# gergely-flamich/relative-entropy-coding

Measured on AMD Instinct MI355X. Metric: encoded latents/sec, higher is better.
Workload: dtype f32

## Files before the change

relative-entropy-coding_amd/csrc/irec_fast_common.h:

```cpp
#pragma once
#include <hip/hip_runtime.h>
#include <stdint.h>

#include "irec_device.h"
#include "irec_kernels.h"

namespace irec {

__device__ __forceinline__ int64_t src_index(const EncArgs &A, int64_t base, int32_t pos, int d) {
  return base + (A.perm ? (int64_t)A.perm[pos + d] : (int64_t)(pos + d));
}

__device__ __forceinline__ void commit_table_stamps(const EncArgs &A) {
  if (A.ws_head != nullptr && blockIdx.x == 0 && threadIdx.x < 4 * WS_STAMP_WORDS)
    A.ws_head[WS_STAMP_WORD + threadIdx.x] = A.ws_head[WS_PENDING_WORD + threadIdx.x];
}

__device__ __forceinline__ void plain_table_rows(int64_t seed, int32_t S, int32_t D, int32_t K_tab, const uint16_t *__restrict__ dlog4r,
                                                 uint16_t *__restrict__ tab, int64_t wg, int64_t n_wg) {
  const int Dp = (D + 3) & ~3;
  const int64_t per_step = (int64_t)S * Dp;
  const int64_t total = per_step * K_tab;
  for (int64_t q = (wg * 256 + threadIdx.x) * 4; q < total; q += n_wg * 256 * 4) {
    const int t = (int)(q / per_step);
    const int64_t rem = q - (int64_t)t * per_step;
    const int s = (int)(rem / Dp), d0 = (int)(rem - (int64_t)s * Dp);
    const StepSeed ss = make_step_seed(seed + t);
    uint16_t v[4];
#pragma unroll
    for (int i = 0; i < 4; ++i) v[i] = (d0 + i < D) ? dlog4r[draw_rm1(ss, (uint64_t)s * (uint64_t)D + (uint64_t)(d0 + i))] : (uint16_t)0;
    *reinterpret_cast<uint2 *>(tab + q) = make_uint2((uint32_t)v[0] | ((uint32_t)v[1] << 16), (uint32_t)v[2] | ((uint32_t)v[3] << 16));
  }
}

__device__ __forceinline__ unsigned long long stamp_now() { return __builtin_amdgcn_s_memtime(); }

template <int MB, int CPW = 32, int NC = 64>
struct SmallLdsT {
  static constexpr int CANDS = NC;
  static constexpr int CP = CPW;
  union {
    unsigned long long wb[32];
    unsigned long long cand[NC];
  };
  int32_t sel_s[MB], sel_b[MB];
  uint32_t sel_bo[MB];
  int32_t hsum[2][MB];
  uint32_t beta4[2][MB];
  int32_t misc[8];
  union {
    double gpart[4];
    float cpart[4][CPW];
  };
  float Cb[CPW];
};
using SmallLds = SmallLdsT<64>;
constexpr size_t SMALL_LDS_BYTES = (sizeof(SmallLds) + 15) & ~(size_t)15;

struct NoPost { __device__ __forceinline__ void operator()(int, int32_t, int32_t, uint32_t) const {} };
template <bool QUICK>
__device__ __forceinline__ uint32_t kth_largest_lane_max(uint32_t M, int Bnew) {
  uint32_t cnt_gt = 0u;
#pragma unroll
  for (int l = 0; l < 64; ++l) cnt_gt += (uint32_t)__builtin_amdgcn_readlane((int)M, l) > M ? 1u : 0u;
  if constexpr (!QUICK) {
    uint32_t T = cnt_gt < (uint32_t)Bnew ? M : 0xFFFFFFFFu;
    T = 0xFFFFFFFFu - (uint32_t)wave_max_u64((unsigned long long)(0xFFFFFFFFu - T));
    return T;
  }
  uint32_t T = 0u;
  for (int c = Bnew <= 64 ? Bnew - 1 : 63; c >= 0; --c) {
    const unsigned long long hit = __ballot(cnt_gt == (uint32_t)c);
    if (hit) { T = (uint32_t)__builtin_amdgcn_readlane((int)M, (int)__builtin_ctzll(hit)); break; }
  }
  return T;
}

template <bool QUICK, class SM, class Post>
__device__ __forceinline__ bool rank_survivors(SM *sm, uint32_t C, int Bnew, int Bcur, int tid, Post &&post) {
  constexpr int NQ = SM::CANDS / 64;
  if (C > (uint32_t)SM::CANDS || C < (uint32_t)Bnew) return false;
  if (C > 64u) {
    if constexpr (NQ > 1) {
      uint32_t mk[NQ], mf[NQ];
#pragma unroll
      for (int q = 0; q < NQ; ++q) {
        const uint32_t at = (uint32_t)(q * 64 + tid);
        const unsigned long long v = at < C ? sm->cand[at] : 0ull;
        mk[q] = (uint32_t)(v >> 32); mf[q] = (uint32_t)v;
      }
      uint32_t T2 = 0u;
      for (int bit = 31; bit >= 0; --bit) {
        const uint32_t tryT = T2 | (1u << bit);
        uint32_t cnt = 0u;
#pragma unroll
        for (int q = 0; q < NQ; ++q) cnt += (uint32_t)__popcll(__ballot(mk[q] >= tryT));
        if (cnt >= (uint32_t)Bnew) T2 = tryT;
      }
      uint32_t base = 0u;
#pragma unroll
      for (int q = 0; q < NQ; ++q) {
        const bool in = mk[q] >= T2 && mk[q] != 0u;
        const unsigned long long mask = __ballot(in);
        const uint32_t pos = base + __builtin_amdgcn_mbcnt_hi((uint32_t)(mask >> 32), __builtin_amdgcn_mbcnt_lo((uint32_t)mask, 0u));
        if (in && pos < 64u) sm->cand[pos] = ((unsigned long long)mk[q] << 32) | mf[q];
        base += (uint32_t)__popcll(mask);
      }
      C = (uint32_t)__builtin_amdgcn_readfirstlane((int)base);
      if (C > 64u) return false;
    } else {
      return false;
    }
  }
  const unsigned long long mine = tid < (int)C ? sm->cand[tid] : 0ull;
  const uint32_t mk1 = (uint32_t)(mine >> 32), mf1 = (uint32_t)mine;
  uint32_t rank = 0u;
  if constexpr (!QUICK) {
    for (uint32_t l = 0; l < C; ++l) {
      const uint32_t ok_ = (uint32_t)__builtin_amdgcn_readlane((int)mk1, (int)l);
      const uint32_t of_ = (uint32_t)__builtin_amdgcn_readlane((int)mf1, (int)l);
      rank += (ok_ > mk1 || (ok_ == mk1 && of_ < mf1)) ? 1u : 0u;
    }
  } else {
  const uint32_t nf1 = ~mf1;
  const unsigned long long mp = ((unsigned long long)mk1 << 32) | nf1;
#pragma unroll
  for (int l0 = 0; l0 < 64; l0 += 8) {
    if ((uint32_t)l0 < C) {
#pragma unroll
      for (int l = l0; l < l0 + 8; ++l) rank += (uint32_t)__builtin_amdgcn_readlane((int)mk1, l) > mk1 ? 1u : 0u;
    }
  }
  volatile unsigned long long *slot = sm->cand;
  if (tid < (int)C) slot[rank] = (unsigned long long)tid;
  const bool lost = tid < (int)C && slot[rank] != (unsigned long long)tid;
  if (__ballot(lost)) {
    rank = 0u;
// ... 377 lines not shown
__device__ __forceinline__ int rsn_owner(int lane) {
  int idx = 0, cnt = N0, n = N0;
#pragma unroll
  for (int dist = 32; dist >= 1; dist >>= 1) {
    if (n >= 2) {
      const int H = (n + 1) / 2;
      if (lane & dist) { idx += H; cnt -= H; } else cnt = cnt < H ? cnt : H;
      n = H;
    }
  }
  return cnt >= 1 ? idx : -1;
}

typedef float rs_f2 __attribute__((ext_vector_type(2)));
__device__ __forceinline__ float reduce_scatter_20(rs_f2 (&a)[10], int lane) {
  float w[5];
#pragma unroll
  for (int k = 0; k < 5; ++k) {
    float px = a[k].x, py = a[k].y, qx = a[k + 5].x, qy = a[k + 5].y;
    swap32(px, qx); swap32(py, qy);
    a[k] = (rs_f2){px, py} + (rs_f2){qx, qy};
  }
#pragma unroll
  for (int k = 0; k < 2; ++k) {
    float px = a[k].x, py = a[k].y, qx = a[k + 2].x, qy = a[k + 2].y;
    swap16(px, qx); swap16(py, qy);
    a[k] = (rs_f2){px, py} + (rs_f2){qx, qy};
  }
  float tx = a[4].x, ty = a[4].y;
  swap16(tx, ty);
  w[0] = a[0].x; w[1] = a[0].y; w[2] = a[1].x; w[3] = a[1].y; w[4] = tx + ty;
  float r0, r1, r2, q0, q1;
  asm("s_nop 1\n\t"
      "v_add_f32_dpp %0, %3, %3 row_ror:8 row_mask:0xf bank_mask:0x3\n\t"
      "v_add_f32_dpp %1, %4, %4 row_ror:8 row_mask:0xf bank_mask:0x3\n\t"
      "v_add_f32_dpp %2, %5, %5 row_ror:8 row_mask:0xf bank_mask:0xf\n\t"
      "v_add_f32_dpp %0, %6, %6 row_ror:8 row_mask:0xf bank_mask:0xc\n\t"
      "v_add_f32_dpp %1, %7, %7 row_ror:8 row_mask:0xf bank_mask:0xc"
      : "=&v"(r0), "=&v"(r1), "=&v"(r2) : "v"(w[0]), "v"(w[1]), "v"(w[2]), "v"(w[3]), "v"(w[4]));
  asm("s_nop 1\n\t"
      "v_add_f32_dpp %0, %2, %2 row_shl:4 row_mask:0xf bank_mask:0x5\n\t"
      "v_add_f32_dpp %1, %3, %3 row_shl:4 row_mask:0xf bank_mask:0xf\n\t"
      "v_add_f32_dpp %0, %4, %4 row_shr:4 row_mask:0xf bank_mask:0xa"
      : "=&v"(q0), "=&v"(q1) : "v"(r0), "v"(r1), "v"(r2));
  float s0, s1, tot;
  asm("s_nop 1\n\t"
      "v_add_f32_dpp %0, %2, %2 quad_perm:[2,3,0,1] row_mask:0xf bank_mask:0xf\n\t"
      "v_add_f32_dpp %1, %3, %3 quad_perm:[2,3,0,1] row_mask:0xf bank_mask:0xf"
      : "=&v"(s0), "=&v"(s1) : "v"(q0), "v"(q1));
  const float kept = (lane & 2) ? s1 : s0;
  asm("s_nop 1\n\t"
      "v_add_f32_dpp %0, %1, %1 quad_perm:[1,0,3,2] row_mask:0xf bank_mask:0xf"
      : "=&v"(tot) : "v"(kept));
  return tot;
}
__device__ __forceinline__ int rs20_owner(int lane) {
  int o5 = 0, cnt = 5, n = 5;
#pragma unroll
  for (int dist = 8; dist >= 1; dist >>= 1) {
    if (n >= 2) {
      const int H = (n + 1) / 2;
      if (lane & dist) { o5 += H; cnt -= H; } else cnt = cnt < H ? cnt : H;
      n = H;
    }
  }
  if (cnt < 1) return -1;
  const int hi16 = (lane >> 4) & 1;
  const int v10 = o5 < 4 ? o5 + 4 * hi16 : 8 + hi16;
  return v10 + ((lane & 32) ? 10 : 0);
}

typedef __attribute__((address_space(3))) const float lds_cfloat;
__device__ __forceinline__ float lds_abs_f32(uint32_t byte_addr) { return *(lds_cfloat *)(uintptr_t)(byte_addr); }

template <int NB, bool TABLE>
struct FastCfg {
  static constexpr int RW = NB <= 10 ? 64 : 32;
  static constexpr int SPC = RW / NB;
  static_assert(SPC >= 1, "NB too large");
};

__host__ __device__ inline size_t fast_ws_bytes(int NB, int max_K) {
  const size_t bp = (((size_t)(max_K > 0 ? max_K : 1) * NB * 4) + 255) & ~(size_t)255;
  return bp + (size_t)5 * FAST_MAX_DIM * 4 + (size_t)2 * NB * FAST_MAX_DIM * 4;
}

}
```

relative-entropy-coding_amd/csrc/irec_team.hip:

```cpp
#include <hip/hip_runtime.h>
#include <algorithm>
#include <stdint.h>
#include <stdio.h>

#include "irec_device.h"
#include "irec_kernels.h"
#include "irec_fast_common.h"
#include "irec_team_common.h"

#ifndef IREC_GANG_ABLATE
#define IREC_GANG_ABLATE 0
#endif
#ifndef IREC_PK_ADDR
#define IREC_PK_ADDR 1
#endif
#if defined(IREC_TEAM_MARGIN_TU) || defined(IREC_TEAM_GANG_TU)
#define IREC_TEAM_AUX_TU 1
#endif
namespace irec {

__host__ __device__ constexpr int team_mb(int NB) { return NB <= 32 ? 32 : 64; }
template <int NB> using TeamLdsT = SmallLdsT<(NB <= 32 ? 32 : 64), (NB <= 32 ? 32 : 64), (NB <= 32 ? 64 : 512)>;
__host__ __device__ inline size_t team_small_bytes(int NB) {
  return NB <= 32 ? ((sizeof(TeamLdsT<32>) + 15) & ~(size_t)15) : ((sizeof(TeamLdsT<64>) + 15) & ~(size_t)15);
// ... 56 lines not shown
  const int S = A.S, B = A.B;
  const int lane = threadIdx.x & 63;
  const int wave_wg = __builtin_amdgcn_readfirstlane((int)(threadIdx.x >> 6));
  const int team = wave_wg / NWT, wave_t = wave_wg % NWT;
  const int wave = wave_t & 3, bs = wave_t >> 2;
  const int b_lo = bs * NBW;
  const int tid = (int)threadIdx.x - team * NT;
  const int PS = NB == 10 ? team_row(NB, B) : NB;
  const int SP = MULTI_PASS ? team_s_pass(NB, S, TEAMS, CMAX, PASSES, PS) : S;
  const bool keys_lds = !MULTI_PASS || team_keys_in_lds(NB, S, TEAMS, PASSES, PS);
  constexpr bool KEYS_ALIAS = TEAMS >= 3 && NB == 20 && !PASSES;
  const size_t key_lds_bytes = (keys_lds && !KEYS_ALIAS) ? team_key_bytes(PS, S) : 0;
  char *tbase = smem + T3_BYTES + (size_t)team * team_lds_one(NB, S, SP, TEAMS, PASSES, PS);
  float *part_s = reinterpret_cast<float *>(tbase);
  TeamLds *sm = reinterpret_cast<TeamLds *>(tbase + team_part_bytes(PS, SP) + key_lds_bytes);
  uint32_t *bar_word = reinterpret_cast<uint32_t *>(tbase + team_part_bytes(PS, SP) + key_lds_bytes + TEAM_SMALL_BYTES);
  double *gpart = sm->gpart;
  int32_t *sel_s = sm->sel_s, *sel_b = sm->sel_b;
  int32_t *hsum = &sm->hsum[0][0];
  uint32_t *beta4 = &sm->beta4[0][0];
  int32_t *misc = sm->misc;
  float *cpart_s = &sm->cpart[0][0];
  const uint16_t *dlog_s = A.dlog4r;
  const int rs_p = rsn_owner<RW>(lane);
  const int rs_p20 = RW == 20 ? rs20_owner(lane) : -1;
  const int rs_c = rsn_owner<NBW>(lane);

  if ((uint32_t)(uintptr_t)(__attribute__((address_space(3))) char *)smem != 0u) __builtin_trap();
  commit_table_stamps(A);
  constexpr bool CAN_SHARE = SHARE && TEAMS >= 2 && BS == 1 && !PASSES && !ONE;
  const int Wsh = (CAN_SHARE && A.coop_W > 1) ? A.coop_W : 1;
  const int64_t n_whole = Wsh > 1 ? (A.tsplit_first < A.n_blocks ? A.tsplit_first : A.n_blocks) : A.n_blocks;
  const int64_t n_slots = n_whole + (A.n_blocks - n_whole) * Wsh;
  const int64_t n_static = (int64_t)TEAMS * (int64_t)gridDim.x < n_slots ? (int64_t)TEAMS * (int64_t)gridDim.x : n_slots;
  constexpr bool CAN_PLACE = NB == 20 && TEAMS == 2 && BS == 1 && !PASSES && !ONE;
  const bool placed = CAN_PLACE && A.row_cost != nullptr && n_static == n_slots;
  const int64_t lo_rank = (int64_t)gridDim.x < n_whole ? (int64_t)gridDim.x : n_whole;
  int32_t placed_row = -1;
  if (placed) {
    uint32_t *cs = reinterpret_cast<uint32_t *>(smem);
    const int n = (int)A.n_blocks;
    for (int k = (int)threadIdx.x; k < n; k += TEAMS * NT) cs[k] = A.row_cost[k];
    if ((int)threadIdx.x < TEAMS) cs[n + (int)threadIdx.x] = 0xFFFFFFFFu;
    int want[TEAMS];
#pragma unroll
    for (int tm = 0; tm < TEAMS; ++tm) {
      const int64_t u = (int64_t)tm * (int64_t)gridDim.x + (int64_t)blockIdx.x;
      want[tm] = u >= n_static ? -1 : u < lo_rank ? (int)u : n - 1 - (int)((u - lo_rank) / (u < n_whole ? 1 : Wsh));
    }
    __syncthreads();
    for (int i = (int)threadIdx.x; i < n; i += TEAMS * NT) {
      const uint32_t ci = cs[i];
      int rk = 0;
#pragma unroll 8
      for (int j = 0; j < n; ++j) rk += cs[j] < ci ? 1 : 0;
#pragma unroll
      for (int tm = 0; tm < TEAMS; ++tm)
        if (rk == want[tm]) cs[n + tm] = (uint32_t)i;
    }
    __syncthreads();
    placed_row = (int32_t)cs[n + team];
    __syncthreads();
  }
  {
    float *l3 = reinterpret_cast<float *>(smem);
    for (int k = (int)threadIdx.x; k < (int)IREC_PM1; k += TEAMS * NT) {
      const float v = A.lut2[k];
      l3[k] = v; l3[k + IREC_PM1] = v; l3[k + 2 * IREC_PM1] = v;
    }
    if (tid == 0) *bar_word = 0u;
  }
  __syncthreads();
  TeamBarrier tsync{bar_word, 0u, (uint32_t)NWT};

  char *slab = A.ws + ((size_t)blockIdx.x * TEAMS + team) * A.ws_per_wg;
  const size_t key_glb_bytes = keys_lds ? 0 : ((team_key_bytes(PS, S) + 255) & ~(size_t)255);
  uint32_t *key_s = KEYS_ALIAS ? reinterpret_cast<uint32_t *>(tbase)
                    : keys_lds ? reinterpret_cast<uint32_t *>(tbase + team_part_bytes(PS, SP))
                               : reinterpret_cast<uint32_t *>(slab + A.ws_per_wg - key_glb_bytes);
  int32_t *bp = reinterpret_cast<int32_t *>(slab);
  float *beams_g = reinterpret_cast<float *>(slab + A.ws_per_wg - key_glb_bytes - (size_t)2 * NB * FAST_MAX_DIM * 4);
  float *stats_g = beams_g - 3 * FAST_MAX_DIM;
  float *park_g = stats_g - 2 * FAST_MAX_DIM;
  constexpr bool PARK = SHORT;
  constexpr bool LATE_G = false;

#ifdef IREC_TEAM_STAMPS
  unsigned long long st_acc[12] = {0, 0, 0, 0, 0, 0, 0, 0, 0, 0, 0, 0};
  unsigned long long st_prev = __builtin_amdgcn_s_memtime();
  const unsigned long long st_t0 = st_prev, st_r0 = __builtin_amdgcn_s_memrealtime();
#endif
  bool first_block = true;
  int steal = 0;
  for (;;) {
    tsync();
    if (tid == 0) {
      int64_t r;
      if (first_block) {
        r = (int64_t)team * (int64_t)gridDim.x + (int64_t)blockIdx.x;
        r = r < n_static ? (placed ? r : xcd_static_row(r, n_static, (int)gridDim.x)) : n_slots;
      } else r = placed ? n_slots : xcd_pull_row(A, n_static, n_slots, steal);
      misc[0] = (int32_t)r;
      misc[6] = 0;
    }
    first_block = false;
    tsync();
    const int64_t slot = misc[0];
    TSTAMP(0);
    if (slot >= n_slots) break;
    int64_t blk = slot < n_whole ? slot : n_whole + (slot - n_whole) / Wsh;
    const int64_t xrow = slot < n_whole ? 0 : (slot - n_whole) / Wsh;
    const int qsh = slot < n_whole ? 0 : (int)((slot - n_whole) % Wsh);
    const int Wrow = slot < n_whole ? 1 : Wsh;
    if (placed) {
      blk = placed_row;
      if (blk < 0 || blk >= A.n_blocks) __builtin_trap();
    }
    if (Wrow > 1 && A.coop_test_orphan && qsh != 0) continue;
    const int D = A.block_dim[blk];
    const int64_t base = A.block_base[blk];
    const int32_t pos = A.block_pos[blk];
    const uint16_t *tab = nullptr;
#pragma unroll
    for (int q = 0; q < 4; ++q)
      if (A.tab_dim[q] == D) tab = A.tab[q];
    if (D < 1 || D > FAST_MAX_DIM || tab == nullptr) {
      if (tid == 0 && qsh == 0) A.out_K[blk] = -1;
      continue;
    }
    const int Dp = (D + 3) & ~3;
    const int NG = (D + 255) >> 8;
    const int NSW = NW / NG;
    const bool active = wave < NG * NSW;
    const int g = wave % NG, sw = wave / NG;
    const int NSWe = NSW * Wrow, swe = sw * Wrow + qsh;
    const int d0 = g * 256 + lane * 4;

    float c[4];
    bool valid[4];
    float own_dmu[4], own_vq[4], own_vp[4];
    const bool own_stats = active && sw == 0 && bs == 0 && TEAMS < 3 && !SHORT;
    double klacc = 0.0;
#pragma unroll
    for (int i = 0; i < 4; ++i) {
      const int d = d0 + i;
      valid[i] = d < D;
      c[i] = 0.f;
      const int64_t ixi = valid[i] ? src_index(A, base, pos, d) : src_index(A, base, pos, 0);
      float st3[3] = {0.f, 1.f, 1.f};
      if (valid[i] && active && sw == 0 && bs == 0) {
        const float mq_ = A.q_loc[ixi], sq_ = A.q_scale[ixi], mp_ = A.p_loc[ixi], sp_ = A.p_scale[ixi];
        klacc = klacc + kl_dim(mq_, sq_, mp_, sp_);
        st3[0] = mq_ - mp_; st3[1] = sq_ * sq_; st3[2] = sp_ * sp_;
      }
      own_dmu[i] = st3[0]; own_vq[i] = st3[1]; own_vp[i] = st3[2];
      if (active && sw == 0 && bs == 0 && (NSW > 1 || BS > 1 || TEAMS >= 3)) {
        stats_g[d0 + i] = st3[0]; stats_g[FAST_MAX_DIM + d0 + i] = st3[1]; stats_g[2 * FAST_MAX_DIM + d0 + i] = st3[2];
      }
    }
    {
      const double gs = wave_tree_sum(klacc);
      if (sw == 0 && bs == 0 && active && lane == 0) gpart[g] = gs;
      tsync();
      if (tid == 0) {
        double tot = gpart[0];
        for (int gg = 1; gg < NG; ++gg) tot = tot + gpart[gg];
        const int32_t K = num_aux((float)tot, A.omega);
        misc[1] = K;
        if (qsh == 0) A.out_K[blk] = K;
        hsum[0] = 0;
        beta4[0] = 0u;
        if constexpr (MARGIN) { if (qsh == 0) margin_write(A.out_margin, blk, MarginAcc()); }
      }
      tsync();
    }
    const int K = misc[1];
    MarginAcc macc;
    if (K > A.max_K || K > A.K_limit) continue;
    if (K > A.K_tab) {
      if (tid == 0 && qsh == 0) atomicAdd(A.defer_count, 1u);
      continue;
    }
    if (K == 0) {
      if (active && sw == 0 && bs == 0 && qsh == 0) {
#pragma unroll
        for (int i = 0; i < 4; ++i)
          if (valid[i]) { const int64_t ixo = src_index(A, base, pos, d0 + i); A.out_sample[ixo] = 0.f + A.p_loc[ixo]; }
      }
      continue;
    }

    float sa[4], cH[4];
    float G[NBW][4];
    auto step_consts = [&](int t_next, float (&m)[4], float (&cA)[4], float (&cBv)[4]) {
      const float rho = A.rho[K - 1 - t_next];
      float dmu_[4], vq_[4], vp_[4];
      if (own_stats) {
#pragma unroll
        for (int i = 0; i < 4; ++i) { dmu_[i] = own_dmu[i]; vq_[i] = own_vq[i]; vp_[i] = own_vp[i]; }
      } else {
        const float4 q0 = *reinterpret_cast<const float4 *>(stats_g + d0);
        const float4 q1 = *reinterpret_cast<const float4 *>(stats_g + FAST_MAX_DIM + d0);
        const float4 q2 = *reinterpret_cast<const float4 *>(stats_g + 2 * FAST_MAX_DIM + d0);
        dmu_[0] = q0.x; dmu_[1] = q0.y; dmu_[2] = q0.z; dmu_[3] = q0.w;
        vq_[0] = q1.x; vq_[1] = q1.y; vq_[2] = q1.z; vq_[3] = q1.w;
        vp_[0] = q2.x; vp_[1] = q2.y; vp_[2] = q2.z; vp_[3] = q2.w;
      }
#pragma unroll
      for (int i = 0; i < 4; ++i) {
        const StepConst sc = step_constants(rho, dmu_[i], vq_[i], vp_[i], c[i]);
        sa[i] = valid[i] ? sc.sa : 0.f; cH[i] = valid[i] ? sc.H : 0.f;
        m[i] = valid[i] ? sc.m : 0.f; cA[i] = valid[i] ? sc.A : 0.f; cBv[i] = valid[i] ? sc.Bv : 0.f;
        c[i] = c[i] + sc.a;
        __builtin_amdgcn_sched_barrier(0);
      }
    };
    auto park = [&]() {
      if (PARK && active) {
        *reinterpret_cast<float4 *>(park_g + d0) = make_float4(c[0], c[1], c[2], c[3]);
        *reinterpret_cast<float4 *>(park_g + FAST_MAX_DIM + d0) = make_float4(sa[0], sa[1], sa[2], sa[3]);
      }
    };
    auto unpark = [&]() {
      if (PARK && active) {
        asm volatile("" ::: "memory");
        const float4 pc = *reinterpret_cast<const float4 *>(park_g + d0);
        const float4 ps = *reinterpret_cast<const float4 *>(park_g + FAST_MAX_DIM + d0);
        c[0] = pc.x; c[1] = pc.y; c[2] = pc.z; c[3] = pc.w;
        sa[0] = ps.x; sa[1] = ps.y; sa[2] = ps.z; sa[3] = ps.w;
      }
    };
    {
      float m[4], cA[4], cBv[4];
      step_consts(0, m, cA, cBv);
      park();
      float cacc = 0.f;
#pragma unroll
      for (int b = 0; b < NBW; ++b)
#pragma unroll
        for (int i = 0; i < 4; ++i) G[b][i] = 0.f;
#pragma unroll
      for (int i = 0; i < 4; ++i) {
        if (bs == 0) G[0][i] = beam_G(0.f, m[i], cA[i], cBv[i], sa[i]);
        cacc = beam_C_term(cacc, 0.f, m[i], cA[i], cBv[i]);
      }
      const float cg = wave_tree_sum(cacc);
      if (active && sw == 0 && bs == 0 && lane == 0) cpart_s[g * TEAM_MB + 0] = cg;
    }

    TSTAMP(1);
    bool abandoned = false;
    int cur = 0, Bcur = 1;
    uint32_t bv_cur = 0u;
    for (int t = 0; t < K; ++t) {
#ifdef IREC_TEAM_STAMPS
      st_acc[11] += 1ull;
#endif
      const uint16_t *tab_tu = tab + (size_t)t * S * Dp;
      const uint32_t tab_lo = (uint32_t)(d0 < Dp ? d0 : Dp - 4);
      const uint16_t *tab_t = tab_tu + tab_lo;
      uint32_t bet[NBW];
      {
#pragma unroll
        for (int b = 0; b < NBW; ++b) bet[b] = (uint32_t)__builtin_amdgcn_readlane((int)bv_cur, b_lo + b);
      }
      const int nlive = Bcur - b_lo < 0 ? 0 : (Bcur - b_lo < NBW ? Bcur - b_lo : NBW);

      const int N = S * Bcur;
      for (int s_base = 0; s_base < S; s_base += SP) {
      const int s_end = s_base + SP < S ? s_base + SP : S;
      const int Sp = s_end - s_base;
#ifdef IREC_ABLATE_SCORING
      if (false) {
#else
      if (active && Bcur > 1 && (nlive == NBW || 2 * nlive >= NBW)) {
        const int n_mine = Sp > swe ? (Sp - swe + NSWe - 1) / NSWe : 0;
        const int n_chunks = (n_mine + SPC - 1) / SPC;
        auto row = [&](int m) {
          uint2 r = make_uint2(0u, 0u);
          if (m < n_mine) r = *reinterpret_cast<const uint2 *>(tab_tu + ((uint32_t)(s_base + m * NSWe + swe) * (uint32_t)Dp + tab_lo));
          return r;
        };
        uint2 ap_cur[SPC], ap_nxt[SPC];
#pragma unroll
        for (int cc = 0; cc < SPC; ++cc) { ap_cur[cc] = row(cc); ap_nxt[cc] = row(SPC + cc); }
#define IREC_AL(CC, I) ((((I) & 2) ? (((I) & 1) ? (ap_cur[CC].y >> 16) : (ap_cur[CC].y & 0xFFFFu)) : (((I) & 1) ? (ap_cur[CC].x >> 16) : (ap_cur[CC].x & 0xFFFFu))) << 2)
        typedef float f2 __attribute__((ext_vector_type(2)));
        constexpr int NP = NBW / 2;
        constexpr int NQ = 4 * SPC;
        static_assert(NBW % 2 == 0, "beams are processed in pairs");
        constexpr int NH = SHORT ? 2 : 1;
        constexpr int HP = NP / NH;
        constexpr int NQH = NQ * NH;
        static_assert(NP % NH == 0 && NQH % 2 == 0, "granules must tile the slots and alternate buffers cleanly");
        f2 zz[2][HP];
#if IREC_PK_ADDR
        f2 betf[NP];
#pragma unroll
        for (int k = 0; k < NP; ++k) betf[k] = (f2){__uint_as_float(bet[2 * k]), __uint_as_float(bet[2 * k + 1])};
#define IREC_ISSUE(Z, AD, K0) do { const float adf_ = __uint_as_float(AD); const f2 ad2_ = {adf_, adf_}; \
                               _Pragma("unroll") for (int k = 0; k < HP; ++k) { const f2 a2_ = ad2_ + betf[(K0) + k]; \
                                 Z[k].x = lds_abs_f32(__float_as_uint(a2_.x)); Z[k].y = lds_abs_f32(__float_as_uint(a2_.y)); } \
                               __builtin_amdgcn_sched_barrier(0); } while (0)
#else
#define IREC_ISSUE(Z, AD, K0) do { _Pragma("unroll") for (int k = 0; k < HP; ++k) { Z[k].x = lds_abs_f32((AD) + bet[2 * ((K0) + k)]); Z[k].y = lds_abs_f32((AD) + bet[2 * ((K0) + k) + 1]); } \
                               __builtin_amdgcn_sched_barrier(0); } while (0)
#endif
#define IREC_CONSUME(Z, I, ACC, K0) do { _Pragma("unroll") for (int k = 0; k < HP; ++k) asm volatile("" : "+v"(Z[k])); \
                                f2 t2_[HP]; \
                                _Pragma("unroll") for (int k = 0; k < HP; ++k) { \
                                  const f2 h2 = {cH[I], cH[I]}, g2 = {G[2 * ((K0) + k)][I], G[2 * ((K0) + k) + 1][I]}; \
                                  t2_[k] = __builtin_elementwise_fma(h2, Z[k], g2); }  \
                                _Pragma("unroll") for (int k = 0; k < HP; ++k)  \
                                  ACC[(K0) + k] = __builtin_elementwise_fma(t2_[k], Z[k], ACC[(K0) + k]); \
// ... 238 lines not shown
#pragma unroll
            for (int gg = 0; gg < 4; ++gg) cbv[q][gg] = cpart_s[(gg < NG ? gg : 0) * TEAM_MB + b];
          }
          if (KEYS_ALIAS && Bcur != NB) {
#pragma unroll
            for (int q = 0; q < MK; ++q)
#pragma unroll
              for (int gg = 0; gg < 4; ++gg) asm volatile("" : "+v"(pr[q][gg]));
            tsync();
          }
          unsigned long long *xg = nullptr;
          if (CAN_SHARE && Wrow > 1)
            xg = reinterpret_cast<unsigned long long *>(A.coop_xch) + ((size_t)(t & 1) * COOP_MAX_BLOCKS + (size_t)xrow) * COOP_KEYS;
          const unsigned long long tag64 = (unsigned long long)(uint32_t)(t + 1) << 32;
          uint32_t foreign = 0u;
#pragma unroll
          for (int q = 0; q < MK; ++q) {
            float sc = pr[q][0];
            if (NG > 1) sc = sc + pr[q][1];
            if (NG > 2) sc = sc + pr[q][2];
            if (NG > 3) sc = sc + pr[q][3];
            float cb = cbv[q][0];
            if (NG > 1) cb = cb + cbv[q][1];
            if (NG > 2) cb = cb + cbv[q][2];
            if (NG > 3) cb = cb + cbv[q][3];
            const int f = q * NT + tid;
            if (f < Np) {
              bool mine = true;
              if (CAN_SHARE && Wrow > 1) {
                const int s_ = Bcur == NB ? f / NB : f / Bcur;
                mine = ((s_ % NSWe) % Wrow) == qsh;
              }
              if (mine) {
                const uint32_t key = score_key(sc + cb);
                key_s[f_base + f] = key;
                if (CAN_SHARE && Wrow > 1) __hip_atomic_store(&xg[f], tag64 | (unsigned long long)key, __ATOMIC_RELAXED, __HIP_MEMORY_SCOPE_AGENT);
              } else foreign |= 1u << q;
            }
          }
          if (CAN_SHARE && Wrow > 1) {
            const uint32_t tag = (uint32_t)(t + 1);
            const unsigned long long t0 = __builtin_amdgcn_s_memrealtime();
            int32_t bad = 0;
            for (uint32_t turn = 1; foreign != 0u; ++turn) {
              unsigned long long gq[MK];
#pragma unroll
              for (int q = 0; q < MK; ++q)
                gq[q] = (foreign >> q) & 1u ? __hip_atomic_load(&xg[q * NT + tid], __ATOMIC_RELAXED, __HIP_MEMORY_SCOPE_AGENT) : 0ull;
#pragma unroll
              for (int q = 0; q < MK; ++q)
                if (((foreign >> q) & 1u) && (uint32_t)(gq[q] >> 32) == tag) { key_s[f_base + q * NT + tid] = (uint32_t)gq[q]; foreign &= ~(1u << q); }
              if (foreign == 0u || (turn & 63u) != 0u) continue;
              if (__hip_atomic_load(A.coop_err, __ATOMIC_RELAXED, __HIP_MEMORY_SCOPE_AGENT) != 0u) { bad = 1; break; }
              if (__builtin_amdgcn_s_memrealtime() - t0 > COOP_GIVE_UP_TICKS) {
                __hip_atomic_store(A.coop_err, 1u, __ATOMIC_RELAXED, __HIP_MEMORY_SCOPE_AGENT);
                bad = 1; break;
              }
            }
            if (bad) misc[6] = 1;
          }
        }
      }
      if (s_end < S) tsync();
      }
      if (CAN_SHARE && Wrow > 1) {
        tsync();
        if (misc[6]) { abandoned = true; break; }
      }
      const int Bnew = B < N ? B : N;
      TSTAMP(4);
#ifdef IREC_ABLATE_SELECT
      tsync();
      if (tid < Bnew) { sel_s[tid] = tid % S; sel_b[tid] = tid % Bcur; sm->sel_bo[tid] = beta4[cur * TEAM_MB + tid % Bcur];
                        hsum[(cur ^ 1) * TEAM_MB + tid] = 0; beta4[(cur ^ 1) * TEAM_MB + tid] = 0u; }
      tsync();
#else
      constexpr bool QUICK_SEL = TEAMS <= 2 && !MULTI_PASS;
      if constexpr (QUICK_SEL) __builtin_assume(N <= 1024);
      select_topB_sync<NT, QUICK_SEL>(key_s, N, Bnew, Bcur, sm, tid, tsync, nullptr, [&](int j, int32_t sp_, int32_t bp_, uint32_t key_) {
        const int32_t nh = (int32_t)((uint32_t)hsum[cur * TEAM_MB + bp_] + (uint32_t)sp_ * (uint32_t)(69 + t));
        hsum[(cur ^ 1) * TEAM_MB + j] = nh;
        sm->sel_bo[j] = beta4[cur * TEAM_MB + bp_];
        bp[(size_t)t * NB + j] = (sp_ << 6) | bp_;
        if constexpr (MARGIN) margin_stash(sm, j, key_);
      });
      if constexpr (MARGIN) {
        if (tid < 64) margin_step(key_s, N, Bnew, Bcur, sm, lane, t == K - 1, macc);
        tsync();
      }
#endif
      TSTAMP(5);
      const bool last = (t == K - 1);
      __builtin_amdgcn_s_setprio(2);
      uint32_t bv_new;
      {
        const int32_t nh = hsum[(cur ^ 1) * TEAM_MB + (lane < Bnew ? lane : 0)];
        bv_new = dlog_s[hash_from_sum(nh) - 1u];
      }
#ifdef IREC_ABLATE_UPDATE
      if (false) {
#else
      if (active) {
#endif
        unpark();
        const float sa_t[4] = {sa[0], sa[1], sa[2], sa[3]};
        const float *bold = beams_g + ((size_t)cur * NB) * FAST_MAX_DIM + d0;
        float *bnew = beams_g + ((size_t)(cur ^ 1) * NB) * FAST_MAX_DIM + d0;
#pragma unroll
        for (int j = 0; j < NBW; ++j)
#pragma unroll
          for (int i = 0; i < 4; ++i) G[j][i] = 0.f;
        float m[4], cA[4], cBv[4];
#pragma unroll
        for (int i = 0; i < 4; ++i) { m[i] = 0.f; cA[i] = 0.f; cBv[i] = 0.f; }
        float cacc[rsn_room(NBW)];
#pragma unroll
        for (int j = 0; j < rsn_room(NBW); ++j) cacc[j] = 0.f;
        constexpr int UB = (TEAMS >= 3 || BS >= 2) ? 5 : NBW;
        const int Bupd = last ? 1 : Bnew;
        const int32_t v_sp = sel_s[lane < Bnew ? lane : 0], v_bp = sel_b[lane < Bnew ? lane : 0];
        const uint32_t v_bo = sm->sel_bo[lane < Bnew ? lane : 0];
#pragma unroll
        for (int j0 = 0; j0 < NBW; j0 += UB) {
          uint2 apv[UB];
          float4 obv4[UB];
          uint32_t bet_old[UB];
#pragma unroll
          for (int u = 0; u < UB; ++u) {
            const int jj = j0 + u, j = b_lo + jj;
            apv[u] = make_uint2(0u, 0u);
            obv4[u] = make_float4(0.f, 0.f, 0.f, 0.f);
            bet_old[u] = 0u;
            if (jj < NBW && j < Bupd) {
              const int32_t sp_ = __builtin_amdgcn_readlane(v_sp, j);
              const int32_t bp_ = __builtin_amdgcn_readlane(v_bp, j);
              bet_old[u] = (uint32_t)__builtin_amdgcn_readlane((int)v_bo, j);
              apv[u] = *reinterpret_cast<const uint2 *>(tab_t + (size_t)sp_ * Dp);
#ifndef IREC_ABLATE_SLAB
              if (t) obv4[u] = *reinterpret_cast<const float4 *>(bold + (size_t)bp_ * FAST_MAX_DIM);
#endif
            }
          }
          if (j0 == 0 && !last) { step_consts(t + 1, m, cA, cBv); park(); }
          if (j0 == 0) TSTAMP(9);
          constexpr int YB = 5;
          float zy[YB][4];
#pragma unroll
          for (int u = 0; u < UB; ++u) {
            if (u % YB == 0) {
#pragma unroll
              for (int v = 0; v < YB; ++v) {
                const int uu = u + v < UB ? u + v : UB - 1;
                const uint32_t al[4] = {(apv[uu].x & 0xFFFFu) << 2, (apv[uu].x >> 16) << 2, (apv[uu].y & 0xFFFFu) << 2, (apv[uu].y >> 16) << 2};
#pragma unroll
                for (int i = 0; i < 4; ++i) zy[v][i] = lds_abs_f32(al[i] + bet_old[uu]);
              }
            }
            const int jj = j0 + u, j = b_lo + jj;
            if (jj < NBW && j < Bupd) {
              const float obv[4] = {obv4[u].x, obv4[u].y, obv4[u].z, obv4[u].w};
              float nb[4];
#pragma unroll
              for (int i = 0; i < 4; ++i) {
                const float y = sa_t[i] * zy[u % YB][i];
                nb[i] = obv[i] + y;
              }
              if (last) {
                if (j == 0 && sw == 0 && qsh == 0) {
#pragma unroll
                  for (int i = 0; i < 4; ++i)
                    if (valid[i]) {
                      const int64_t ixo = src_index(A, base, pos, d0 + i);
                      A.out_sample[ixo] = nb[i] + A.p_loc[ixo];
                    }
                }
              } else {
#ifndef IREC_ABLATE_SLAB
                if (sw == 0) *reinterpret_cast<float4 *>(bnew + (size_t)j * FAST_MAX_DIM) = make_float4(nb[0], nb[1], nb[2], nb[3]);
#endif
                if constexpr (LATE_G) {
#pragma unroll
                  for (int i = 0; i < 4; ++i) G[jj][i] = nb[i];
                } else {
#pragma unroll
                  for (int i = 0; i < 4; ++i) {
                    G[jj][i] = beam_G(nb[i], m[i], cA[i], cBv[i], sa[i]);
                    cacc[jj] = beam_C_term(cacc[jj], nb[i], m[i], cA[i], cBv[i]);
                  }
                }
              }
            }
          }
          __builtin_amdgcn_sched_barrier(0);
        }
        if constexpr (LATE_G) {
          if (!last) {
#pragma unroll
            for (int jj = 0; jj < NBW; ++jj) {
              if (b_lo + jj < Bnew) {
#pragma unroll
                for (int i = 0; i < 4; ++i) {
                  const float nbv = G[jj][i];
                  G[jj][i] = beam_G(nbv, m[i], cA[i], cBv[i], sa[i]);
                  cacc[jj] = beam_C_term(cacc[jj], nbv, m[i], cA[i], cBv[i]);
                }
              }
              __builtin_amdgcn_sched_barrier(0);
            }
          }
        }
        TSTAMP(10);
        if (!last) {
          const float ctot = reduce_scatter_n<NBW>(cacc, lane);
          if (sw == 0 && (lane & 1) == 0 && rs_c >= 0 && b_lo + rs_c < Bnew) cpart_s[g * TEAM_MB + b_lo + rs_c] = ctot;
        }
      }
      TSTAMP(6);
      __builtin_amdgcn_s_setprio(0);
      if (tid < Bnew) beta4[(cur ^ 1) * TEAM_MB + tid] = bv_new;
      bv_cur = bv_new;
      cur ^= 1;
      Bcur = Bnew;
    }
    tsync();
    if (abandoned) {
      if (tid == 0 && qsh == 0) A.out_K[blk] = -2;
      continue;
    }
    if (tid == 0 && qsh == 0) {
      int j = 0;
      for (int t = K - 1; t >= 0; --t) {
        const int32_t v = __builtin_nontemporal_load(&bp[(size_t)t * NB + j]);
        A.out_indices[blk * (int64_t)A.max_K + t] = v >> 6;
        j = v & 63;
      }
      if constexpr (MARGIN) margin_write(A.out_margin, blk, macc);
    }
    TSTAMP(8);
  }
#ifdef IREC_TEAM_STAMPS
  if (A.dbg && lane == 0)
    for (int k = 0; k < 12; ++k) A.dbg[((size_t)blockIdx.x * (TEAMS * BS * 4) + wave_wg) * 16 + k] = st_acc[k];
  if (A.dbg && lane == 0) {
    A.dbg[((size_t)blockIdx.x * (TEAMS * BS * 4) + wave_wg) * 16 + 12] = __builtin_amdgcn_s_memtime() - st_t0;
    A.dbg[((size_t)blockIdx.x * (TEAMS * BS * 4) + wave_wg) * 16 + 13] = __builtin_amdgcn_s_memrealtime() - st_r0;
  }
#endif
}

#ifndef IREC_TEAM_MARGIN_TU
constexpr int CHUNK_MAX_DIM = 1 << 22;
__host__ __device__ inline size_t chunk_ws_bytes(int NB, int dpad, int max_K) {
  return (size_t)(6 + 2 * NB) * dpad * 4 + ((((size_t)(max_K > 0 ? max_K : 1) * NB * 4) + 255) & ~(size_t)255);
}
__host__ __device__ inline size_t chunk_lds_one(int NB, int NBP, int S) {
  return team_part_bytes(NBP, S) + team_key_bytes(NB, S) + team_small_bytes(NB) + 16;
}
__host__ __device__ inline size_t chunk_lds_total(int NB, int NBP, int S, int teams) { return T3_BYTES + (size_t)teams * chunk_lds_one(NB, NBP, S); }

template <int NB, int NBP, int TEAMS, bool GANG = false>
__global__ __launch_bounds__(TEAMS * TEAM_NT, 1) void encode_chunk_kernel(EncArgs A) {
  using TeamLds = TeamLdsT<NB>;
  constexpr int TEAM_MB = team_mb(NB);
  constexpr size_t TEAM_SMALL_BYTES = (sizeof(TeamLds) + 15) & ~(size_t)15;
  constexpr int NT = TEAM_NT;
  constexpr int SPC = NBP <= 10 ? 20 / NBP : 1;
  constexpr int RW = NBP * SPC;
  static_assert(NB % NBP == 0 && (NBP == 10 || NBP == 16 || NBP == 20) && NB <= 60, "chunked encoder: passes of 10, 16 or 20 beams, at most 60 beam slots (6-bit back-pointers)");
  extern __shared__ __attribute__((aligned(16))) char smem[];
  const int S = A.S, B = A.B;
  const int lane = threadIdx.x & 63;
  const int wave_wg = __builtin_amdgcn_readfirstlane((int)(threadIdx.x >> 6));
  const int team = wave_wg / TEAM_NW, g = wave_wg % TEAM_NW;
  const int tid = (int)threadIdx.x - team * NT;
  char *tbase = smem + T3_BYTES + (size_t)team * chunk_lds_one(NB, NBP, S);
  float *part_s = reinterpret_cast<float *>(tbase);
  float *run_s = reinterpret_cast<float *>(tbase + team_part_bytes(NBP, S));
  uint32_t *key_s = reinterpret_cast<uint32_t *>(run_s);
  TeamLds *sm = reinterpret_cast<TeamLds *>(tbase + team_part_bytes(NBP, S) + team_key_bytes(NB, S));
  uint32_t *bar_word = reinterpret_cast<uint32_t *>(tbase + team_part_bytes(NBP, S) + team_key_bytes(NB, S) + TEAM_SMALL_BYTES);
  double *gpart = sm->gpart;
  int32_t *sel_s = sm->sel_s, *sel_b = sm->sel_b;
  int32_t *hsum = &sm->hsum[0][0];
  uint32_t *beta4 = &sm->beta4[0][0];
  int32_t *misc = sm->misc;
  float *cpart_s = &sm->cpart[0][0];
  float *Cb_s = sm->Cb;
  const uint16_t *dlog_s = A.dlog4r;
  const int rs_p = rsn_owner<RW>(lane), rs_c = rsn_owner<NBP>(lane);
  const int rs_p20 = RW == 20 ? rs20_owner(lane) : -1;
  double *kl_tot = reinterpret_cast<double *>(sm->wb);

  if ((uint32_t)(uintptr_t)(__attribute__((address_space(3))) char *)smem != 0u) __builtin_trap();
  commit_table_stamps(A);
  {
    float *l3 = reinterpret_cast<float *>(smem);
    for (int k = (int)threadIdx.x; k < (int)IREC_PM1; k += TEAMS * NT) {
      const float v = A.lut2[k];
      l3[k] = v; l3[k + IREC_PM1] = v; l3[k + 2 * IREC_PM1] = v;
    }
    if (tid == 0) *bar_word = 0u;
  }
// ... 1015 lines not shown
```

Before: 178,400.

## Skip beam slab store at penultimate step and rebuild beams from grandparent on last step

At step K-2 the kernel no longer writes the new beam positions to the global slab. It records each beam's ancestor index in LDS and saves the step scale to a new keep buffer. At the final step it recomputes the parent beam from the grandparent slab row plus the previous step's table entry. This removes one full slab write round per block in exchange for extra table loads, LDS lookups and arithmetic on the last step, plus a slightly larger workspace.

After: 176,500 (median of 2 runs). 0.989x the previous value.

```diff
diff --git a/relative-entropy-coding_amd/csrc/irec_fast_common.h b/relative-entropy-coding_amd/csrc/irec_fast_common.h
--- a/relative-entropy-coding_amd/csrc/irec_fast_common.h
+++ b/relative-entropy-coding_amd/csrc/irec_fast_common.h
@@ -52,7 +52,10 @@
     double gpart[4];
     float cpart[4][CPW];
   };
-  float Cb[CPW];
+  union {
+    float Cb[CPW];
+    int32_t anc[CPW];
+  };
 };
 using SmallLds = SmallLdsT<64>;
 constexpr size_t SMALL_LDS_BYTES = (sizeof(SmallLds) + 15) & ~(size_t)15;
@@ -596,7 +599,7 @@
 
 __host__ __device__ inline size_t fast_ws_bytes(int NB, int max_K) {
   const size_t bp = (((size_t)(max_K > 0 ? max_K : 1) * NB * 4) + 255) & ~(size_t)255;
-  return bp + (size_t)5 * FAST_MAX_DIM * 4 + (size_t)2 * NB * FAST_MAX_DIM * 4;
-}
-
-}
+  return bp + (size_t)6 * FAST_MAX_DIM * 4 + (size_t)2 * NB * FAST_MAX_DIM * 4;
+}
+
+}
diff --git a/relative-entropy-coding_amd/csrc/irec_team.hip b/relative-entropy-coding_amd/csrc/irec_team.hip
--- a/relative-entropy-coding_amd/csrc/irec_team.hip
+++ b/relative-entropy-coding_amd/csrc/irec_team.hip
@@ -162,6 +162,7 @@
   float *beams_g = reinterpret_cast<float *>(slab + A.ws_per_wg - key_glb_bytes - (size_t)2 * NB * FAST_MAX_DIM * 4);
   float *stats_g = beams_g - 3 * FAST_MAX_DIM;
   float *park_g = stats_g - 2 * FAST_MAX_DIM;
+  float *keep_g = park_g - FAST_MAX_DIM;
   constexpr bool PARK = SHORT;
   constexpr bool LATE_G = false;
 
@@ -310,6 +311,7 @@
         sa[0] = ps.x; sa[1] = ps.y; sa[2] = ps.z; sa[3] = ps.w;
       }
     };
+    auto rebuilt = [&](int t_) { return t_ >= 1 && t_ == K - 1; };
     {
       float m[4], cA[4], cBv[4];
       step_consts(0, m, cA, cBv);
@@ -714,6 +716,7 @@
         hsum[(cur ^ 1) * TEAM_MB + j] = nh;
         sm->sel_bo[j] = beta4[cur * TEAM_MB + bp_];
         bp[(size_t)t * NB + j] = (sp_ << 6) | bp_;
+        if (t == K - 2) sm->anc[j] = (sp_ << 6) | bp_;
         if constexpr (MARGIN) margin_stash(sm, j, key_);
       });
       if constexpr (MARGIN) {
@@ -738,6 +741,9 @@
         const float sa_t[4] = {sa[0], sa[1], sa[2], sa[3]};
         const float *bold = beams_g + ((size_t)cur * NB) * FAST_MAX_DIM + d0;
         float *bnew = beams_g + ((size_t)(cur ^ 1) * NB) * FAST_MAX_DIM + d0;
+        const bool rebuild = rebuilt(t);
+        const bool store = !last && !rebuilt(t + 1);
+        if (!last && !store && sw == 0) *reinterpret_cast<float4 *>(keep_g + d0) = make_float4(sa_t[0], sa_t[1], sa_t[2], sa_t[3]);
 #pragma unroll
         for (int j = 0; j < NBW; ++j)
 #pragma unroll
@@ -752,29 +758,67 @@
         const int Bupd = last ? 1 : Bnew;
         const int32_t v_sp = sel_s[lane < Bnew ? lane : 0], v_bp = sel_b[lane < Bnew ? lane : 0];
         const uint32_t v_bo = sm->sel_bo[lane < Bnew ? lane : 0];
+        int32_t v_an = 0;
+        uint32_t v_bg = 0u;
+        if (rebuild) {
+          v_an = sm->anc[v_bp];
+          if (t >= 2) v_bg = beta4[(cur ^ 1) * TEAM_MB + (v_an & 63)];
+        }
 #pragma unroll
         for (int j0 = 0; j0 < NBW; j0 += UB) {
           uint2 apv[UB];
           float4 obv4[UB];
           uint32_t bet_old[UB];
+          uint2 ppv[UB];
+          uint32_t bet_gp[UB];
 #pragma unroll
           for (int u = 0; u < UB; ++u) {
             const int jj = j0 + u, j = b_lo + jj;
             apv[u] = make_uint2(0u, 0u);
             obv4[u] = make_float4(0.f, 0.f, 0.f, 0.f);
             bet_old[u] = 0u;
+            ppv[u] = make_uint2(0u, 0u);
+            bet_gp[u] = 0u;
             if (jj < NBW && j < Bupd) {
               const int32_t sp_ = __builtin_amdgcn_readlane(v_sp, j);
               const int32_t bp_ = __builtin_amdgcn_readlane(v_bp, j);
               bet_old[u] = (uint32_t)__builtin_amdgcn_readlane((int)v_bo, j);
               apv[u] = *reinterpret_cast<const uint2 *>(tab_t + (size_t)sp_ * Dp);
+              if (rebuild) {
+                const int32_t an = __builtin_amdgcn_readlane(v_an, j);
+                ppv[u] = *reinterpret_cast<const uint2 *>(tab_t - (size_t)S * Dp + (size_t)(an >> 6) * Dp);
+                if (t >= 2) {
+                  bet_gp[u] = (uint32_t)__builtin_amdgcn_readlane((int)v_bg, j);
 #ifndef IREC_ABLATE_SLAB
-              if (t) obv4[u] = *reinterpret_cast<const float4 *>(bold + (size_t)bp_ * FAST_MAX_DIM);
+                  obv4[u] = *reinterpret_cast<const float4 *>(bnew + (size_t)(an & 63) * FAST_MAX_DIM);
+#endif
+                }
+              }
+#ifndef IREC_ABLATE_SLAB
+              else if (t) obv4[u] = *reinterpret_cast<const float4 *>(bold + (size_t)bp_ * FAST_MAX_DIM);
 #endif
             }
           }
           if (j0 == 0 && !last) { step_consts(t + 1, m, cA, cBv); park(); }
           if (j0 == 0) TSTAMP(9);
+          if (rebuild) {
+            const float4 sk = *reinterpret_cast<const float4 *>(keep_g + d0);
+            const float sa_p[4] = {sk.x, sk.y, sk.z, sk.w};
+#pragma unroll
+            for (int u = 0; u < UB; ++u) {
+              const uint32_t al[4] = {(ppv[u].x & 0xFFFFu) << 2, (ppv[u].x >> 16) << 2, (ppv[u].y & 0xFFFFu) << 2, (ppv[u].y >> 16) << 2};
+              float zp[4], x[4];
+#pragma unroll
+              for (int i = 0; i < 4; ++i) zp[i] = lds_abs_f32(al[i] + bet_gp[u]);
+              const float ob[4] = {obv4[u].x, obv4[u].y, obv4[u].z, obv4[u].w};
+#pragma unroll
+              for (int i = 0; i < 4; ++i) {
+                const float y = sa_p[i] * zp[i];
+                x[i] = ob[i] + y;
+              }
+              obv4[u] = make_float4(x[0], x[1], x[2], x[3]);
+            }
+          }
           constexpr int YB = 5;
           float zy[YB][4];
 #pragma unroll
@@ -808,7 +852,7 @@
                 }
               } else {
 #ifndef IREC_ABLATE_SLAB
-                if (sw == 0) *reinterpret_cast<float4 *>(bnew + (size_t)j * FAST_MAX_DIM) = make_float4(nb[0], nb[1], nb[2], nb[3]);
+                if (sw == 0 && store) *reinterpret_cast<float4 *>(bnew + (size_t)j * FAST_MAX_DIM) = make_float4(nb[0], nb[1], nb[2], nb[3]);
 #endif
                 if constexpr (LATE_G) {
 #pragma unroll
@@ -849,7 +893,7 @@
       }
       TSTAMP(6);
       __builtin_amdgcn_s_setprio(0);
-      if (tid < Bnew) beta4[(cur ^ 1) * TEAM_MB + tid] = bv_new;
+      if (!last && tid < Bnew) beta4[(cur ^ 1) * TEAM_MB + tid] = bv_new;
       bv_cur = bv_new;
       cur ^= 1;
       Bcur = Bnew;
```
